# esi-neuroscience/syncopy

Measured on AMD Instinct MI355X. Metric: trials/sec for mtmfft+coherence (256 ch x 4096 samples, 7 DPSS tapers, full CSD), higher is better.
Workload: dtype f32 transforms; CSD operands fp16 hi+lo (22-bit), f32 accumulate; 1 GPU; BASELINE configs[2]: connectivityanalysis method='coh', AR(2) AnalogData, 256 ch x 4096 samp x 1000 trials per GPU, tapsmofrq=1 Hz (7 DPSS tapers), polyremoval=0, output='abs', inputs resident in HBM; trials_per_gpu=1000, channels=256, samples=4096, tapers=7, freqs=2049, batch=1000, fft_kernel=mtmfft_quad_kernel<12, 2, 2, false> + seq_mean_kernel

## Files before the change

include/spyhip.h:

```cpp
#ifndef SPYHIP_H
#define SPYHIP_H

#include <stddef.h>
#include <stdint.h>

#ifdef __cplusplus
extern "C" {
#endif

typedef struct spyhip_ctx spyhip_ctx;
typedef struct spyhip_fft_plan spyhip_fft_plan;
typedef struct spyhip_cwt_plan spyhip_cwt_plan;
typedef struct spyhip_queue spyhip_queue;

enum spyhip_output {
    SPYHIP_OUT_POW = 0,
    SPYHIP_OUT_ABS = 1,
    SPYHIP_OUT_FOURIER = 2,
    SPYHIP_OUT_REAL = 3,
    SPYHIP_OUT_IMAG = 4,
    SPYHIP_OUT_ANGLE = 5,
    SPYHIP_OUT_ABSREAL = 6,
    SPYHIP_OUT_ABSIMAG = 7
};

enum spyhip_detrend { SPYHIP_DETREND_NONE = -1, SPYHIP_DETREND_CONSTANT = 0, SPYHIP_DETREND_LINEAR = 1 };

int spyhip_version(void);
const char* spyhip_last_error(void);
int spyhip_ctx_create(int device, spyhip_ctx** ctx);
int spyhip_ctx_destroy(spyhip_ctx* ctx);
int spyhip_ctx_trim(spyhip_ctx* ctx);
int spyhip_ctx_set_stream(spyhip_ctx* ctx, void* stream);
int spyhip_ctx_synchronize(spyhip_ctx* ctx);

int spyhip_alloc(spyhip_ctx* ctx, size_t bytes, void** ptr_d);
int spyhip_free(spyhip_ctx* ctx, void* ptr_d);
int spyhip_memset(spyhip_ctx* ctx, void* ptr_d, int value, size_t bytes);
int spyhip_upload(spyhip_ctx* ctx, void* dst_d, const void* src, size_t bytes);
int spyhip_download(spyhip_ctx* ctx, void* dst, const void* src_d, size_t bytes);

int spyhip_queue_upload(spyhip_ctx* ctx, const float* data, int64_t nrows, int nchan, const int64_t* sampleinfo,
                        int ntrials, spyhip_queue** queue);
int spyhip_queue_destroy(spyhip_queue* queue);
const float* spyhip_queue_data(const spyhip_queue* queue);
int spyhip_queue_segments(const spyhip_queue* queue, const int64_t** start_d, const int64_t** stop_d, int* ntrials);

#define SPYHIP_UNIQUE_ID_BYTES 128
int spyhip_comm_unique_id(void* id_out);
int spyhip_comm_init(spyhip_ctx* ctx, const void* id, int rank, int nranks);
int spyhip_comm_destroy(spyhip_ctx* ctx);
int spyhip_comm_info(const spyhip_ctx* ctx, int* rank, int* nranks);
int spyhip_allreduce_csd(spyhip_ctx* ctx, void* acc_d, int nfreq, int nchan);
int spyhip_allreduce(spyhip_ctx* ctx, void* buf_d, int64_t n, int dtype);

int spyhip_fft_plan_create(spyhip_ctx* ctx, int nsig, int nfft, int nchan, int ntaper,
                           const double* tapers, double scale, int detrend, int demean_taper,
                           const int32_t* freq_idx, int nfsel, int output, int keeptapers,
                           spyhip_fft_plan** plan);
int spyhip_fft_plan_destroy(spyhip_fft_plan* plan);
int spyhip_fft_exec(spyhip_fft_plan* plan, const float* data_d, int64_t ld,
                    const int32_t* chan_idx_d, const int64_t* seg_start_d, const int64_t* seg_lo_d,
                    const int64_t* seg_hi_d, int nseg, void* out_d);
int spyhip_fft_plan_set_blocked(spyhip_fft_plan* plan, int on);
int spyhip_fft_plan_set_precision(spyhip_fft_plan* plan, int reference);
int spyhip_fft_plan_set_reference_mean(spyhip_fft_plan* plan, int on);
int spyhip_fft_plan_set_absmax(spyhip_fft_plan* plan, float* absmax_d);
const char* spyhip_fft_plan_kernel_name(const spyhip_fft_plan* plan);

int spyhip_csd_accumulate(spyhip_ctx* ctx, const void* spec_d, int64_t nrows, int nfreq, int nchan,
                          void* acc_d);
int spyhip_csd_set_phase_exact(spyhip_ctx* ctx, int on);
int spyhip_csd_accumulate_split(spyhip_ctx* ctx, const void* spec_d, int64_t nrows, int nfreq, int nchan,
                                void* acc_d, const float* absmax_d);
int spyhip_csd_accumulate_split_range(spyhip_ctx* ctx, const void* spec_d, int64_t nrows, int nfreq, int nchan,
                                      void* acc_d, const float* absmax_d, int f0, int nf);
int spyhip_csd_split_fallbacks(spyhip_ctx* ctx, int* count);
int spyhip_csd_accumulate_blocked(spyhip_ctx* ctx, const void* spec_d, int64_t nrows, int nfreq, int nchan,
                                  void* acc_d);
int spyhip_csd_tril_pack(spyhip_ctx* ctx, const void* acc_d, int nfreq, int nchan, void* packed_d);
int spyhip_csd_tril_unpack(spyhip_ctx* ctx, const void* packed_d, int nfreq, int nchan, void* acc_d);
int spyhip_csd_finalize(spyhip_ctx* ctx, void* acc_d, int nfreq, int nchan, double scale);

int spyhip_coh_normalize(spyhip_ctx* ctx, const void* csd_d, int nfreq, int nchan, int output,
                         void* out_d);

int spyhip_coh_from_accumulator(spyhip_ctx* ctx, const void* acc_d, int nfreq, int nchan, double scale, int output,
                                void* out_d);

int spyhip_cwt_plan_create_sl(spyhip_ctx* ctx, int nsig, int nchan, int nscales, const double* scales, double dt,
                              double cycles, double k_sd, int detrend, int output, const int32_t* tpos, int ntime_out,
                              spyhip_cwt_plan** out);
int spyhip_slt_combine(spyhip_ctx* ctx, void* acc_d, const void* spec_d, int64_t nrows, int nscales, int nsub, int s0,
                       int nchan, const double* expo, int init, int modulus_only);
int spyhip_spec_convert(spyhip_ctx* ctx, const void* in_d, int64_t n, int output, void* out_d);

int spyhip_ppc_accumulate(spyhip_ctx* ctx, const void* spec_d, int ntrials, int ntaper, int nfreq, int nchan,
                          void* acc_d);
int spyhip_ppc_accumulate_csd(spyhip_ctx* ctx, const void* csd_d, int ntrials, int64_t nelem, void* acc_d);
int spyhip_ppc_finalize(spyhip_ctx* ctx, const void* acc_d, int nfreq, int ni, int nj, int lower_only,
                        int64_t ntrials, void* out_d);

int spyhip_jack_coh_accumulate(spyhip_ctx* ctx, const void* spec_d, int ntrials, int ntaper, int nfreq, int nchan,
                               const void* csd_d, const void* direct_d, int output, int64_t ntrials_total,
                               void* sum_d, void* sum_d2);

int spyhip_ccov_nfft(int nsamples);
int spyhip_ccov_from_accumulator(spyhip_ctx* ctx, const void* acc_d, int nfft, int nchan, int nsamples, double scale,
                                 int norm, void* out_d);
int spyhip_ccov_normalize(spyhip_ctx* ctx, void* cc_d, int nlag, int nchan);

int spyhip_cwt_plan_create(spyhip_ctx* ctx, int nsig, int nchan, int nscales, const double* scales,
                           double dt, double w0, int detrend, int output, const int32_t* tpos,
                           int ntime_out, spyhip_cwt_plan** plan);
int spyhip_cwt_plan_create_family(spyhip_ctx* ctx, int nsig, int nchan, int nscales, const double* scales,
                                  double dt, int family, double p0, double p1, int detrend, int output,
                                  const int32_t* tpos, int ntime_out, spyhip_cwt_plan** plan);
int spyhip_cwt_plan_destroy(spyhip_cwt_plan* plan);
int spyhip_cwt_plan_set_precision(spyhip_cwt_plan* plan, int reference);
// ... 65 lines not shown
```

syncopy_amd/_lib.py:

```python
import ctypes as C
import os

HERE = os.path.dirname(os.path.abspath(__file__))
LIB_PATH = os.path.join(HERE, "libspyhip.so")

_lib = None

c_i32p = C.POINTER(C.c_int32)
c_i64p = C.POINTER(C.c_int64)
c_f32p = C.POINTER(C.c_float)
c_f64p = C.POINTER(C.c_double)
vp = C.c_void_p

SIGNATURES = {
    "spyhip_version": (C.c_int, []),
    "spyhip_last_error": (C.c_char_p, []),
    "spyhip_ctx_create": (C.c_int, [C.c_int, C.POINTER(vp)]),
    "spyhip_ctx_destroy": (C.c_int, [vp]),
    "spyhip_ctx_set_stream": (C.c_int, [vp, vp]),
    "spyhip_ctx_trim": (C.c_int, [vp]),
    "spyhip_ctx_synchronize": (C.c_int, [vp]),
    "spyhip_alloc": (C.c_int, [vp, C.c_size_t, C.POINTER(vp)]),
    "spyhip_free": (C.c_int, [vp, vp]),
    "spyhip_memset": (C.c_int, [vp, vp, C.c_int, C.c_size_t]),
    "spyhip_upload": (C.c_int, [vp, vp, vp, C.c_size_t]),
    "spyhip_download": (C.c_int, [vp, vp, vp, C.c_size_t]),
    "spyhip_queue_upload": (C.c_int, [vp, vp, C.c_int64, C.c_int, c_i64p, C.c_int, C.POINTER(vp)]),
    "spyhip_queue_destroy": (C.c_int, [vp]),
    "spyhip_queue_data": (vp, [vp]),
    "spyhip_queue_segments": (C.c_int, [vp, C.POINTER(vp), C.POINTER(vp), C.POINTER(C.c_int)]),
    "spyhip_comm_unique_id": (C.c_int, [vp]),
    "spyhip_comm_init": (C.c_int, [vp, vp, C.c_int, C.c_int]),
    "spyhip_comm_destroy": (C.c_int, [vp]),
    "spyhip_comm_info": (C.c_int, [vp, C.POINTER(C.c_int), C.POINTER(C.c_int)]),
    "spyhip_allreduce_csd": (C.c_int, [vp, vp, C.c_int, C.c_int]),
    "spyhip_allreduce": (C.c_int, [vp, vp, C.c_int64, C.c_int]),
    "spyhip_fft_plan_set_precision": (C.c_int, [vp, C.c_int]),
    "spyhip_cwt_plan_set_precision": (C.c_int, [vp, C.c_int]),
    "spyhip_cwt_plan_set_direct": (C.c_int, [vp, C.c_int]),
    "spyhip_fft_plan_set_reference_mean": (C.c_int, [vp, C.c_int]),
    "spyhip_fft_plan_create": (C.c_int, [vp, C.c_int, C.c_int, C.c_int, C.c_int, c_f64p, C.c_double, C.c_int,
                                         C.c_int, c_i32p, C.c_int, C.c_int, C.c_int, C.POINTER(vp)]),
    "spyhip_fft_plan_destroy": (C.c_int, [vp]),
    "spyhip_fft_exec": (C.c_int, [vp, vp, C.c_int64, vp, vp, vp, vp, C.c_int, vp]),
    "spyhip_fft_plan_kernel_name": (C.c_char_p, [vp]),
    "spyhip_fft_plan_set_blocked": (C.c_int, [vp, C.c_int]),
    "spyhip_csd_accumulate": (C.c_int, [vp, vp, C.c_int64, C.c_int, C.c_int, vp]),
    "spyhip_csd_set_phase_exact": (C.c_int, [vp, C.c_int]),
    "spyhip_csd_accumulate_split": (C.c_int, [vp, vp, C.c_int64, C.c_int, C.c_int, vp, vp]),
    "spyhip_csd_accumulate_split_range": (C.c_int, [vp, vp, C.c_int64, C.c_int, C.c_int, vp, vp, C.c_int, C.c_int]),
    "spyhip_csd_split_fallbacks": (C.c_int, [vp, C.POINTER(C.c_int)]),
    "spyhip_fft_plan_set_absmax": (C.c_int, [vp, vp]),
    "spyhip_csd_accumulate_blocked": (C.c_int, [vp, vp, C.c_int64, C.c_int, C.c_int, vp]),
    "spyhip_coh_from_accumulator": (C.c_int, [vp, vp, C.c_int, C.c_int, C.c_double, C.c_int, vp]),
    "spyhip_ppc_accumulate": (C.c_int, [vp, vp, C.c_int, C.c_int, C.c_int, C.c_int, vp]),
    "spyhip_ppc_accumulate_csd": (C.c_int, [vp, vp, C.c_int, C.c_int64, vp]),
    "spyhip_ppc_finalize": (C.c_int, [vp, vp, C.c_int, C.c_int, C.c_int, C.c_int, C.c_int64, vp]),
    "spyhip_jack_coh_accumulate": (C.c_int, [vp, vp, C.c_int, C.c_int, C.c_int, C.c_int, vp, vp, C.c_int, C.c_int64,
                                             vp, vp]),
    "spyhip_ccov_nfft": (C.c_int, [C.c_int]),
    "spyhip_ccov_normalize": (C.c_int, [vp, vp, C.c_int, C.c_int]),
    "spyhip_ccov_from_accumulator": (C.c_int, [vp, vp, C.c_int, C.c_int, C.c_int, C.c_double, C.c_int, vp]),
    "spyhip_csd_tril_pack": (C.c_int, [vp, vp, C.c_int, C.c_int, vp]),
    "spyhip_csd_tril_unpack": (C.c_int, [vp, vp, C.c_int, C.c_int, vp]),
    "spyhip_csd_finalize": (C.c_int, [vp, vp, C.c_int, C.c_int, C.c_double]),
    "spyhip_coh_normalize": (C.c_int, [vp, vp, C.c_int, C.c_int, C.c_int, vp]),
    "spyhip_cwt_plan_create": (C.c_int, [vp, C.c_int, C.c_int, C.c_int, c_f64p, C.c_double, C.c_double, C.c_int,
                                         C.c_int, c_i32p, C.c_int, C.POINTER(vp)]),
    "spyhip_cwt_plan_create_sl": (C.c_int, [vp, C.c_int, C.c_int, C.c_int, c_f64p, C.c_double, C.c_double,
                                            C.c_double, C.c_int, C.c_int, c_i32p, C.c_int, C.POINTER(vp)]),
    "spyhip_cwt_plan_create_family": (C.c_int, [vp, C.c_int, C.c_int, C.c_int, c_f64p, C.c_double, C.c_int, C.c_double,
                                                C.c_double, C.c_int, C.c_int, c_i32p, C.c_int, C.POINTER(vp)]),
    "spyhip_slt_combine": (C.c_int, [vp, vp, vp, C.c_int64, C.c_int, C.c_int, C.c_int, C.c_int, c_f64p, C.c_int,
                                     C.c_int]),
    "spyhip_spec_convert": (C.c_int, [vp, vp, C.c_int64, C.c_int, vp]),
    "spyhip_cwt_plan_destroy": (C.c_int, [vp]),
    "spyhip_cwt_exec": (C.c_int, [vp, vp, C.c_int64, vp, vp, vp, vp, C.c_int, vp, C.c_int]),
    "spyhip_granger": (C.c_int, [vp, vp, C.c_int, C.c_int, C.c_double, C.c_int, C.c_double, C.c_double, vp, vp, vp,
                                 c_f64p]),
    "spyhip_granger_last_iterations": (C.c_int, [vp]),
    "spyhip_wilson_cond": (C.c_int, [vp, vp, C.c_int, C.c_int, C.c_double, vp, vp, c_f64p]),
    "spyhip_wilson_init": (C.c_int, [vp, vp, C.c_int, C.c_int, C.c_int, C.c_int, vp, vp]),
    "spyhip_wilson_psi0": (C.c_int, [vp, vp, C.c_int, C.c_int, vp, vp]),
    "spyhip_wilson_g": (C.c_int, [vp, vp, vp, C.c_int, C.c_int, C.c_int, vp, vp]),
    "spyhip_wilson_plus": (C.c_int, [vp, vp, C.c_int, C.c_int64, vp, vp]),
    "spyhip_wilson_update": (C.c_int, [vp, vp, vp, vp, vp, vp, C.c_int, C.c_int, vp, c_f64p]),
    "spyhip_wilson_finish": (C.c_int, [vp, vp, vp, vp, C.c_int, C.c_int, vp, vp, vp, vp]),
    "spyhip_trial_mean_f32": (C.c_int, [vp, vp, vp, C.c_int64, C.c_int64]),
    "spyhip_trial_mean_c64": (C.c_int, [vp, vp, vp, C.c_int64, C.c_int64]),
    "spyhip_axis_nanmean": (C.c_int, [vp, vp, C.c_int64, C.c_int64, C.c_int64, C.c_int, vp]),
    "spyhip_trial_sum": (C.c_int, [vp, vp, vp, C.c_int64, C.c_int64]),
    "spyhip_trial_sum_finalize": (C.c_int, [vp, vp, vp, C.c_int64, C.c_int64, C.c_int]),
    "spyhip_trial_sqdev": (C.c_int, [vp, vp, vp, vp, C.c_int64, C.c_int64, C.c_int]),
# ... 50 lines not shown
```

syncopy_amd/backend.py:

```python
import ctypes as C
import os

import numpy as np
import torch

from . import _lib
from ._lib import SpyHipError, check

OUTPUT_KIND = {"pow": 0, "abs": 1, "fourier": 2, "complex": 2, "real": 3, "imag": 4, "angle": 5,
               "absreal": 6, "absimag": 7}
DETREND = {None: -1, False: -1, 0: 0, 1: 1}

_contexts = {}
_NP_DTYPE = {torch.float32: np.float32, torch.float64: np.float64, torch.complex64: np.complex64,
             torch.complex128: np.complex128, torch.int32: np.int32, torch.int64: np.int64, torch.uint8: np.uint8}


def require_gpu():
    if not torch.cuda.is_available():
        raise SpyHipError("no HIP device visible: syncopy_amd has no CPU fallback (torch.cuda.is_available() is False)")


class Context:

# ... 299 lines not shown
    for ctx in _contexts.values():
        ctx.lib.spyhip_ctx_trim(ctx.handle)
    if torch.cuda.is_available():
        torch.cuda.empty_cache()


def handover_buffer(shape, device, dtype=torch.complex64):
    key = (tuple(shape), str(device), dtype)
    buf = _handover.get(key)
    if buf is None:
        _handover.clear()
        buf = torch.empty(shape, dtype=dtype, device=device)
        _handover[key] = buf
    return buf


USE_BLOCKED_HANDOVER = False


class FFTPlan:

    def __init__(self, nsig, nfft, nchan, tapers, scale, detrend=None, demean_taper=False, freq_idx=None,
                 output="pow", keeptapers=True, device=None, reference_mean=False):
        self.ctx = context(device)
        tapers = np.ascontiguousarray(np.atleast_2d(tapers), dtype=np.float64)
        assert tapers.shape[1] == nsig, (tapers.shape, nsig)
        self.nsig, self.nfft, self.nchan, self.ntaper = int(nsig), int(nfft), int(nchan), tapers.shape[0]
        self.output = output
        self.kind = OUTPUT_KIND[output]
        self.keeptapers = bool(keeptapers)
        nf = self.nfft // 2 + 1
        if freq_idx is None:
            fi_p, self.nfsel = None, nf
        else:
            fi = np.ascontiguousarray(freq_idx, dtype=np.int32)
            fi_p, self.nfsel = fi.ctypes.data_as(_lib.c_i32p), int(fi.size)
        h = C.c_void_p()
        self.ctx.bind_stream()
        check(self.ctx.lib.spyhip_fft_plan_create(
            self.ctx.handle, self.nsig, self.nfft, self.nchan, self.ntaper,
            tapers.ctypes.data_as(_lib.c_f64p), float(scale), DETREND[detrend], int(bool(demean_taper)),
            fi_p, self.nfsel, self.kind, int(self.keeptapers), C.byref(h)), "spyhip_fft_plan_create")
        self.handle = h
        self.kout = self.ntaper if self.keeptapers else 1
        self.out_dtype = torch.complex64 if self.kind == 2 else torch.float32
        self.blocked = False
        self.reference_mean = int(reference_mean)
        if self.reference_mean:
            check(self.ctx.lib.spyhip_fft_plan_set_reference_mean(self.handle, self.reference_mean),
                  "spyhip_fft_plan_set_reference_mean")

    def set_precision(self, reference=True):
        return self.ctx.lib.spyhip_fft_plan_set_precision(self.handle, int(bool(reference))) == 0

    def set_blocked(self, on=True):
        rc = self.ctx.lib.spyhip_fft_plan_set_blocked(self.handle, int(bool(on)))
        if rc == 0:
            self.blocked = bool(on)
        return rc == 0

    @property
    def kernel_name(self):
        return self.ctx.lib.spyhip_fft_plan_kernel_name(self.handle).decode()

    def out_shape(self, nseg):
        if self.blocked:
            return (nseg * self.kout, (self.nchan + 3) // 4, self.nfsel, 4)
        return (nseg, self.kout, self.nfsel, self.nchan)

    def execute(self, data, seg_start, seg_lo=None, seg_hi=None, chan_idx=None, out=None, absmax=None):
        assert data.is_cuda and data.dtype == torch.float32 and data.dim() == 2 and data.is_contiguous()
        dev = data.device
        nseg = int(seg_start.numel())
        if seg_lo is None:
            seg_lo = seg_start
        if seg_hi is None:
            seg_hi = seg_start + self.nsig
        for t in (seg_start, seg_lo, seg_hi):
            assert t.is_cuda and t.dtype == torch.int64 and t.is_contiguous() and t.numel() == nseg
        if chan_idx is not None:
            assert chan_idx.is_cuda and chan_idx.dtype == torch.int32 and chan_idx.numel() == self.nchan
        else:
            assert data.shape[1] >= self.nchan
        if out is None:
            out = torch.empty(self.out_shape(nseg), dtype=self.out_dtype, device=dev)
        else:
            assert out.is_cuda and out.is_contiguous() and out.dtype == self.out_dtype
            assert tuple(out.shape) == self.out_shape(nseg), (tuple(out.shape), self.out_shape(nseg))
        self.ctx.bind_stream()
        tracked = False
        if absmax is not None:
            assert absmax.is_cuda and absmax.dtype == torch.float32 and absmax.numel() == self.nchan and absmax.is_contiguous()
            tracked = self.ctx.lib.spyhip_fft_plan_set_absmax(self.handle, _ptr(absmax)) == 0
        self.tracked_absmax = tracked
        try:
            check(self.ctx.lib.spyhip_fft_exec(self.handle, _ptr(data), int(data.shape[1]), _ptr(chan_idx),
                                               _ptr(seg_start), _ptr(seg_lo), _ptr(seg_hi), nseg, _ptr(out)),
                  "spyhip_fft_exec")
        finally:
            if self.tracked_absmax:
                self.ctx.lib.spyhip_fft_plan_set_absmax(self.handle, None)
        out.spyhip_absmax_tracked = self.tracked_absmax
        return out

    def __del__(self):
        try:
# ... 716 lines not shown
```

syncopy_amd/csrc/mtmfft.hip:

```cpp
#include <algorithm>
#include <cmath>
#include <cstdlib>
#include <string>

#include "spy_common.h"
#include "host_fft.h"
#include "mtmfft_kernel.h"
#include "mtmfft2_kernel.h"
#include "mtmfft_blue_kernel.h"
#include "mtmfft_long.h"
#include "mtmfft_generic.h"
#include "mtmfft_mixed_plan.h"

namespace spyfft {
}
#include "f64_stockham.h"
#include "mtmfft_f64_args.h"
namespace spyfft {
int dec64_launch_a(hipStream_t stream, const F64Args& a, int nfft, int npairs, int outk, bool mean);
int dec64_launch_b(hipStream_t stream, const F64Args& a, int nfft, int npairs, int outk, bool mean);
int dec64_launch_c(hipStream_t stream, const F64Args& a, int nfft, int npairs, int outk, bool mean);
int dec64_launch_d(hipStream_t stream, const F64Args& a, int nfft, int npairs, int outk, bool mean);
int dec64_launch_e(hipStream_t stream, const F64Args& a, int nfft, int npairs, int outk, bool mean);
int dec64_launch_f(hipStream_t stream, const F64Args& a, int nfft, int npairs, int outk, bool mean);
// ... 3 lines not shown
int dec64_launch_j(hipStream_t stream, const F64Args& a, int nfft, int npairs, int outk, bool mean);
int dec64_launch_k(hipStream_t stream, const F64Args& a, int nfft, int npairs, int outk, bool mean);
int dec64_launch_l(hipStream_t stream, const F64Args& a, int nfft, int npairs, int outk, bool mean);
int dec64_launch_m(hipStream_t stream, const F64Args& a, int nfft, int npairs, int outk, bool mean);
int dec64_launch_n(hipStream_t stream, const F64Args& a, int nfft, int npairs, int outk, bool mean);
int dec64_launch_half_a(hipStream_t stream, const F64Args& a, int nfft, int nchan, int outk, bool mean);
int dec64_launch_half_b(hipStream_t stream, const F64Args& a, int nfft, int nchan, int outk, bool mean);
struct Long64Args {
    MtmArgs m;
    const double* tapers64;
    const double2* twM;
    const double2* twN;
    const double2* twP;
    double2* scratch;
    const double* stats;
    const double* wsum;
    int seg0, nsegc;
    int npair;
};
int declong64_group(int M);
int declong64_launch_sub_a(hipStream_t stream, const Long64Args& a, int M, int P, long long nblocks);
int declong64_launch_sub_b(hipStream_t stream, const Long64Args& a, int M, int P, long long nblocks);
int declong64_launch_post(hipStream_t stream, const Long64Args& a, int P, int M, int outk, bool mean);
int f64_any_launch(hipStream_t stream, F64Args a, long long grid, long long chunk, int outk, bool mean);
int dec_launch_a(hipStream_t stream, const MtmArgs& a, int nfft, int nquads, int outk, bool mean);
int dec_launch_b(hipStream_t stream, const MtmArgs& a, int nfft, int nquads, int outk, bool mean);
int dec_launch_c(hipStream_t stream, const MtmArgs& a, int nfft, int nquads, int outk, bool mean);
int dec_launch_d(hipStream_t stream, const MtmArgs& a, int nfft, int nquads, int outk, bool mean);
int dec_launch_e(hipStream_t stream, const MtmArgs& a, int nfft, int nquads, int outk, bool mean);
int dec_launch_f(hipStream_t stream, const MtmArgs& a, int nfft, int nquads, int outk, bool mean);
int dec_launch_g(hipStream_t stream, const MtmArgs& a, int nfft, int nquads, int outk, bool mean);
int dec_launch_h(hipStream_t stream, const MtmArgs& a, int nfft, int nquads, int outk, bool mean);
int dec_launch_i(hipStream_t stream, const MtmArgs& a, int nfft, int nquads, int outk, bool mean);
int dec_launch_j(hipStream_t stream, const MtmArgs& a, int nfft, int nquads, int outk, bool mean);
int dec_launch_k(hipStream_t stream, const MtmArgs& a, int nfft, int nquads, int outk, bool mean);
int dec_launch_l(hipStream_t stream, const MtmArgs& a, int nfft, int nquads, int outk, bool mean);
int dec_launch_c2(hipStream_t stream, const MtmArgs& a, int nquads);
int dec_launch_half_a(hipStream_t stream, const MtmArgs& a, int nfft, int npairs, int outk, bool mean);
int dec_launch_half_b(hipStream_t stream, const MtmArgs& a, int nfft, int npairs, int outk, bool mean);
int dec_launch_half_c(hipStream_t stream, const MtmArgs& a, int nfft, int npairs, int outk, bool mean);
int quad_half_launch(hipStream_t stream, const MtmArgs& a, int npairs, int outk, bool mean);
int declong_group(int M);
int declong_launch_sub_a(hipStream_t stream, const LongArgs& a, int M, int P, long long nblocks);
int declong_launch_sub_b(hipStream_t stream, const LongArgs& a, int M, int P, long long nblocks);
int declong_launch_post(hipStream_t stream, const LongArgs& a, int P, int M, int outk, bool mean);
int mixed_launch(hipStream_t stream, const MtmArgs& a, const MixPlan& g, int threads, size_t lds, unsigned grid, int outk,
                 bool mean);
}

using spyfft::GenPlan;
using spyfft::MtmArgs;

struct spyhip_fft_plan {
    spyhip_ctx* ctx = nullptr;
    int nsig = 0, nfft = 0, nchan = 0, ntaper = 0, nfsel = 0, output = 0, keeptapers = 1;
    int detrend = -1, demean_taper = 0;
    float scale = 1.f;
    bool pow2 = false;
    bool dec = false;
    bool half = false;
    spy::DevBuf<float2> twh;
    bool mixed = false;
    spyfft::MixPlan mix{};
    int mix_threads = 0;
    bool blue = false;
    bool longp = false;
    bool long_direct = false;
    int dl_P = 0, dl_M = 0;
    int l1 = 0, l2 = 0;
    spy::DevBuf<float2> tw1, tw2, twM;
    spy::DevBuf<double> wsum, stats, stats_part;
    spy::DevBuf<float4> scratch;
    size_t stats_cap = 0, scratch_cap = 0;
    int log2n = 0, G = 1;
    GenPlan gen{};
    size_t lds_bytes = 0;
    spy::DevBuf<float> tapers;
    spy::DevBuf<float> tapers_half;
    spy::DevBuf<float2> tw, chirp, bhat;
    spy::DevBuf<int> fpos;
    bool identity_freq = true;
    bool blocked = false;
    unsigned* absmax = nullptr;
    float wnorm = 0.f;
    bool precision64 = false;
    bool f64_any = false;
    bool f64_dec = false;
    int f64_blue = 0;
    bool f64_dl = false;
    bool f64_half = false;
    spy::DevBuf<double2> tw64h;
    spy::DevBuf<double2> tw64_sub, tw64_P, scratch64;
    size_t scratch64_cap = 0;
    spy::DevBuf<double2> chirp64, bhat64;
    spywil::PlusPlan f64_plan{};
    spy::DevBuf<double2> f64_work;
    long long f64_chunk = 0;
    spy::DevBuf<double> tapers64;
    spy::DevBuf<double2> tw64;
    std::string fp32_kernel_name;
    bool ref_mean = false;
    bool seg_f64 = false;
    spy::DevBuf<float> means;
    size_t means_cap = 0;
    spy::DevBuf<float2> xpair;
    size_t xpair_cap = 0;
    std::string kernel_name;
};

namespace {

const double PI = 3.14159265358979323846264338327950288;

std::vector<float2> twiddle_table(int n) {
    std::vector<float2> t(n);
    for (int m = 0; m < n; ++m) {
        const double ang = -2.0 * PI * (double)m / (double)n;
        t[m] = make_float2((float)std::cos(ang), (float)std::sin(ang));
    }
    return t;
}

bool factorize(int n, int* radix, int* nfac) {
    static const int cand[] = {16, 8, 4, 2, 3, 5, 7, 11, 13};
    int k = 0;
    for (int c : cand) {
        while (n % c == 0 && n > 1) {
            if (k >= spyfft::GEN_MAXFAC) return false;
            radix[k++] = c;
            n /= c;
        }
    }
    *nfac = k;
    return n == 1;
}

template <int LOG2N, int G, int OUTK, bool MEAN>
int launch_quad(const spyhip_fft_plan* p, const MtmArgs& a, unsigned grid) {
    using C = spyfft::Cfg2<LOG2N, G>;
    auto kern = spyfft::mtmfft_quad_kernel<LOG2N, G, OUTK, MEAN>;
    SPY_HIP_CHECK(hipFuncSetAttribute(reinterpret_cast<const void*>(kern),
                                      hipFuncAttributeMaxDynamicSharedMemorySize, (int)C::LDS_BYTES));
    MtmArgs b = a;
    b.tapers = p->tapers_half.p;
    if (!b.tapers) { spy::set_error("fft_exec: plan without the pre-scaled taper table"); return -1; }
    hipLaunchKernelGGL(kern, dim3(grid), dim3(C::NTHREADS), C::LDS_BYTES, p->ctx->stream, b);
    SPY_HIP_CHECK(hipGetLastError());
    return 0;
}

template <int LOG2N, int G>
int launch_quad_mode(const spyhip_fft_plan* p, const MtmArgs& a, unsigned grid) {
    const bool mean = !p->keeptapers;
    const int outk = p->output == SPYHIP_OUT_FOURIER ? 2 : (p->output == SPYHIP_OUT_POW ? 0 : 1);
    switch (outk * 2 + (mean ? 1 : 0)) {
        case 0: return launch_quad<LOG2N, G, 0, false>(p, a, grid);
        case 1: return launch_quad<LOG2N, G, 0, true>(p, a, grid);
// ... 441 lines not shown
                    const long long q = (n * n) % (2LL * nfft);
                    const double ang = PI * (double)q / (double)nfft;
                    chirp[n] = make_double2(std::cos(ang), -std::sin(ang));
                    br[n] = std::cos(ang);
                    bi[n] = std::sin(ang);
                    if (n > 0) { br[M - n] = br[n]; bi[M - n] = bi[n]; }
                }
                spy::fft_host(br, bi);
                std::vector<double2> bhat(M);
                for (int i = 0; i < M; ++i) bhat[i] = make_double2(br[i] / M, bi[i] / M);
                if (p->chirp64.upload(chirp, p->ctx->stream) || p->bhat64.upload(bhat, p->ctx->stream)) return -2;
            }
        }
    }
    if (!p->tw64.p) {
        std::vector<double2> t(twlen);
        for (int m = 0; m < twlen; ++m) {
            const double ang = -2.0 * PI * (double)m / (double)twlen;
            t[m] = make_double2(std::cos(ang), std::sin(ang));
        }
        if (p->tw64.upload(t, p->ctx->stream)) return -2;
    }
    if (!p->precision64) p->fp32_kernel_name = p->kernel_name;
    p->precision64 = true;
    char buf[128];
    if (p->f64_half)
        std::snprintf(buf, sizeof buf, "mtmfft_dec64_kernel<HALF of N = %d, %d, %s>", p->nfft,
                      p->output == SPYHIP_OUT_FOURIER ? 2 : (p->output == SPYHIP_OUT_POW ? 0 : 1), p->keeptapers ? "false" : "true");
    else if (p->f64_dl)
        std::snprintf(buf, sizeof buf, "declong64_kernel<%d x %d, %d, %s>", p->dl_P, p->dl_M,
                      p->output == SPYHIP_OUT_FOURIER ? 2 : (p->output == SPYHIP_OUT_POW ? 0 : 1), p->keeptapers ? "false" : "true");
    else if (p->f64_dec)
        std::snprintf(buf, sizeof buf, "mtmfft_dec64_kernel<N = %d, %d, %s>", p->nfft,
                      p->output == SPYHIP_OUT_FOURIER ? 2 : (p->output == SPYHIP_OUT_POW ? 0 : 1), p->keeptapers ? "false" : "true");
    else if (p->f64_blue)
        std::snprintf(buf, sizeof buf, "mtmfft_f64_any_kernel<%d, %s> N=%d (Bluestein, M = %d)",
                      p->output == SPYHIP_OUT_FOURIER ? 2 : (p->output == SPYHIP_OUT_POW ? 0 : 1), p->keeptapers ? "false" : "true",
                      p->nfft, p->f64_blue);
    else
        std::snprintf(buf, sizeof buf, "mtmfft_f64_any_kernel<%d, %s> N=%d",
                      p->output == SPYHIP_OUT_FOURIER ? 2 : (p->output == SPYHIP_OUT_POW ? 0 : 1), p->keeptapers ? "false" : "true",
                      p->nfft);
    p->kernel_name = buf;
    return 0;
}

extern "C" int spyhip_fft_plan_set_reference_mean(spyhip_fft_plan* p, int on) {
    if (!p) { spy::set_error("fft_plan_set_reference_mean: null plan"); return -1; }
    p->ref_mean = on == 1;
    p->seg_f64 = on == 2;
    return 0;
}

extern "C" const char* spyhip_fft_plan_kernel_name(const spyhip_fft_plan* p) {
    return p ? p->kernel_name.c_str() : "";
}

extern "C" int spyhip_fft_exec(spyhip_fft_plan* p, const float* data_d, int64_t ld, const int32_t* chan_idx_d,
                               const int64_t* seg_start_d, const int64_t* seg_lo_d, const int64_t* seg_hi_d,
                               int nseg, void* out_d) {
    if (!p || !data_d || !seg_start_d || !seg_lo_d || !seg_hi_d || !out_d) { spy::set_error("fft_exec: null argument"); return -1; }
    if (nseg <= 0) return 0;
    SPY_HIP_CHECK(hipSetDevice(p->ctx->device));
    MtmArgs a{};
    a.data = data_d; a.ld = ld; a.chan_idx = chan_idx_d;
    a.seg_start = reinterpret_cast<const long long*>(seg_start_d);
    a.seg_lo = reinterpret_cast<const long long*>(seg_lo_d);
    a.seg_hi = reinterpret_cast<const long long*>(seg_hi_d);
    a.nseg = nseg; a.nsig = p->nsig; a.nchan = p->nchan; a.ntaper = p->ntaper;
    a.tapers = p->tapers.p; a.tw = p->tw.p; a.scale = p->scale;
    a.detrend = p->detrend; a.demean_taper = p->demean_taper;
    a.fpos = p->identity_freq ? nullptr : p->fpos.p;
    a.nfsel = p->nfsel; a.out_kind = p->output; a.out = out_d;
    a.blocked = p->blocked ? 1 : 0;
    a.means = nullptr;
    a.seg_f64 = p->seg_f64 ? 1 : 0;
    a.absmax = (p->absmax && !p->blocked) ? p->absmax : nullptr;
    a.wnorm = p->wnorm;
    if (a.absmax && !(p->pow2 && p->log2n <= 13 && !p->precision64)) {
        const int bt = std::min(256, ((p->nchan + 63) / 64) * 64);
        const int ncb = (p->nchan + bt - 1) / bt;
        for (int s0 = 0; s0 < nseg; s0 += 65535) {
            MtmArgs m = a;
            m.seg_start += s0; m.seg_lo += s0; m.seg_hi += s0;
            hipLaunchKernelGGL(spyfft::seg_range_kernel, dim3(ncb, std::min(65535, nseg - s0)), dim3(bt), 0, p->ctx->stream, m);
        }
        SPY_HIP_CHECK(hipGetLastError());
        a.absmax = nullptr;
    }
    if (p->ref_mean && p->detrend == 0) {
        const size_t need = (size_t)nseg * p->nchan;
        if (need > p->means_cap) {
            if (p->means.p) { SPY_HIP_CHECK(hipStreamSynchronize(p->ctx->stream)); (void)hipFree(p->means.p); p->means.p = nullptr; }
            if (p->means.alloc(need)) return -2;
            p->means_cap = need;
        }
        const int bt = std::min(256, ((p->nchan + 63) / 64) * 64);
        const int ncb = (p->nchan + bt - 1) / bt;
        for (int s0 = 0; s0 < nseg; s0 += 65535) {
            MtmArgs m = a;
            m.seg_start += s0; m.seg_lo += s0; m.seg_hi += s0;
            const int ns = std::min(65535, nseg - s0);
            hipLaunchKernelGGL(spyfft::seq_mean_kernel, dim3(ncb, ns), dim3(bt), 0, p->ctx->stream, m,
                               p->means.p + (size_t)s0 * p->nchan);
        }
        SPY_HIP_CHECK(hipGetLastError());
        a.means = p->means.p;
    }
    const int npairs = (p->nchan + 1) / 2;
    if (p->precision64) {
        spyfft::F64Args fa{};
        fa.m = a;
        fa.tapers64 = p->tapers64.p;
        fa.tw64 = p->tw64.p;
        fa.scale64 = (double)p->scale;
        const long long grid = (long long)nseg * npairs;
        const int outk64 = p->output == SPYHIP_OUT_FOURIER ? 2 : (p->output == SPYHIP_OUT_POW ? 0 : 1);
        if (p->f64_half) {
            fa.tw64 = p->tw64h.p;
            fa.tw64_full = p->tw64.p;
            int rc;
            if ((rc = spyfft::dec64_launch_half_a(p->ctx->stream, fa, p->nfft, p->nchan, outk64, !p->keeptapers)) != -100) return rc;
            if ((rc = spyfft::dec64_launch_half_b(p->ctx->stream, fa, p->nfft, p->nchan, outk64, !p->keeptapers)) != -100) return rc;
            spy::set_error("fft_exec: no half-length reference-precision schedule for nfft = %d", p->nfft);
            return -1;
        }
        if (p->f64_dl) {
            spyfft::Long64Args L{};
            a.nfft = p->nfft;
            L.m = a;
            L.tapers64 = p->tapers64.p;
            L.twM = p->tw64_sub.p; L.twN = p->tw64.p; L.twP = p->tw64_P.p;
            L.wsum = p->wsum.p;
            L.npair = npairs;
            const size_t N = (size_t)p->nfft;
            const size_t nstat = (size_t)nseg * p->nchan * (2 + p->ntaper);
            const int nz = p->demean_taper ? p->ntaper + 1 : 1;
            if (nstat > p->stats_cap) {
                if (p->stats.p) { (void)hipFree(p->stats.p); p->stats.p = nullptr; }
                if (p->stats_part.p) { (void)hipFree(p->stats_part.p); p->stats_part.p = nullptr; }
                if (p->stats.alloc(nstat) ||
                    p->stats_part.alloc((size_t)nseg * (p->ntaper + 1) * spyfft::LONG_SPLITS * p->nchan * 2)) return -2;
                p->stats_cap = nstat;
            }
            L.stats = p->stats.p;
            if ((p->detrend >= 0 && !(p->detrend == 0 && a.means)) || p->demean_taper) {
                if (nseg > 65535 || nz * spyfft::LONG_SPLITS > 65535) { spy::set_error("fft_exec: too many segments / tapers per call"); return -1; }
                hipLaunchKernelGGL(spyfft::long_stats_kernel, dim3((p->nchan + 63) / 64, nseg, nz * spyfft::LONG_SPLITS),
                                   dim3(256), 0, p->ctx->stream, a, p->stats_part.p, nz);
                hipLaunchKernelGGL(spyfft::long_stats_final_kernel, dim3((unsigned)(((size_t)nseg * p->nchan + 255) / 256)), dim3(256),
                                   0, p->ctx->stream, a, p->stats_part.p, nz, p->stats.p);
                SPY_HIP_CHECK(hipGetLastError());
            }
            const size_t per_seg = (size_t)npairs * p->ntaper * N;
            size_t chunk = std::max<size_t>(1, std::min<size_t>((size_t)nseg, (((size_t)2 << 30) / sizeof(double2)) / std::max<size_t>(per_seg, 1)));
            if (chunk * per_seg > p->scratch64_cap) {
                if (p->scratch64.p) { (void)hipFree(p->scratch64.p); p->scratch64.p = nullptr; }
                if (p->scratch64.alloc(chunk * per_seg)) return -2;
                p->scratch64_cap = chunk * per_seg;
            }
// ... 257 lines not shown
            L.nsegc = std::min<int>((int)chunk, nseg - s0);
            const long long items = (long long)L.nsegc * L.nquad * p->ntaper;
            int rc = launch_long(p->ctx, L, p->l1, 0, items);
            if (!rc) rc = launch_long(p->ctx, L, p->l2, 1, items);
            if (!rc && !L.direct) rc = launch_long(p->ctx, L, p->l1, 2, items);
            if (rc) return rc;
            switch (outk * 2 + (mean ? 1 : 0)) {
                case 0: rc = launch_long_post<0, false>(p->ctx, L); break;
                case 1: rc = launch_long_post<0, true>(p->ctx, L); break;
                case 2: rc = launch_long_post<1, false>(p->ctx, L); break;
                case 3: rc = launch_long_post<1, true>(p->ctx, L); break;
                case 4: rc = launch_long_post<2, false>(p->ctx, L); break;
                default: rc = launch_long_post<2, true>(p->ctx, L); break;
            }
            if (rc) return rc;
        }
        return 0;
    }
    if (p->blue) {
        a.nfft = p->nfft; a.chirp = p->chirp.p; a.bhat = p->bhat.p;
        const int G = p->G;
        const int nitem = (p->nchan + 3) / 4;
        a.npg = (nitem + G - 1) / G;
        int S = 8 / G; if (S < 1) S = 1; if (S > a.npg) S = a.npg;
        a.S = S;
        a.ncl = (a.npg + S - 1) / S;
        const long long nclusters = (long long)nseg * a.ncl;
        const long long grid = ((nclusters + 7) / 8) * S * 8;
        if (grid > 0x7fffffffLL) { spy::set_error("fft_exec: grid too large (%lld blocks)", grid); return -1; }
        const unsigned g = (unsigned)grid;
        switch (p->log2n) {
            case 8: return launch_blue_mode<8, 16>(p, a, g);
            case 9: return launch_blue_mode<9, 8>(p, a, g);
            case 10: return launch_blue_mode<10, 4>(p, a, g);
            case 11: return launch_blue_mode<11, 2>(p, a, g);
            case 12: return launch_blue_mode<12, 1>(p, a, g);
            case 13: return launch_blue_mode<13, 1>(p, a, g);
            default: spy::set_error("no Bluestein kernel for M=2^%d", p->log2n); return -1;
        }
    }
    const long long grid = (long long)nseg * npairs;
    if (grid > 0x7fffffffLL) { spy::set_error("fft_exec: grid too large (%lld blocks)", grid); return -1; }
    const bool mean = !p->keeptapers;
    const int outk = p->output == SPYHIP_OUT_FOURIER ? 2 : (p->output == SPYHIP_OUT_POW ? 0 : 1);
    switch (outk * 2 + (mean ? 1 : 0)) {
        case 0: return launch_generic<0, false>(p, a, (unsigned)grid);
        case 1: return launch_generic<0, true>(p, a, (unsigned)grid);
        case 2: return launch_generic<1, false>(p, a, (unsigned)grid);
        case 3: return launch_generic<1, true>(p, a, (unsigned)grid);
        case 4: return launch_generic<2, false>(p, a, (unsigned)grid);
        default: return launch_generic<2, true>(p, a, (unsigned)grid);
    }
}
```

Baseline: 49130 trials/s.

## Overlap per-segment mean pass with FFT via chunked side stream

Splits the segment batch into chunks and runs the reference-mean kernel for each chunk on a dedicated non-blocking side stream. Each chunk's transform waits on an event, so the mean pass for later chunks can overlap the FFT of earlier ones instead of running serially in front of the whole batch. The chunk size is derived from CU count and wave geometry, and the path is skipped under graph capture. It adds extra launches and event synchronisation per chunk and shortens each FFT grid, which may hurt occupancy.

```diff
diff --git a/include/spyhip.h b/include/spyhip.h
--- a/include/spyhip.h
+++ b/include/spyhip.h
@@ -65,6 +65,7 @@
 int spyhip_fft_plan_set_blocked(spyhip_fft_plan* plan, int on);
 int spyhip_fft_plan_set_precision(spyhip_fft_plan* plan, int reference);
 int spyhip_fft_plan_set_reference_mean(spyhip_fft_plan* plan, int on);
+int spyhip_fft_plan_set_mean_chunk(spyhip_fft_plan* plan, int nseg);
 int spyhip_fft_plan_set_absmax(spyhip_fft_plan* plan, float* absmax_d);
 const char* spyhip_fft_plan_kernel_name(const spyhip_fft_plan* plan);
 
diff --git a/syncopy_amd/_lib.py b/syncopy_amd/_lib.py
--- a/syncopy_amd/_lib.py
+++ b/syncopy_amd/_lib.py
@@ -39,6 +39,7 @@
     "spyhip_cwt_plan_set_precision": (C.c_int, [vp, C.c_int]),
     "spyhip_cwt_plan_set_direct": (C.c_int, [vp, C.c_int]),
     "spyhip_fft_plan_set_reference_mean": (C.c_int, [vp, C.c_int]),
+    "spyhip_fft_plan_set_mean_chunk": (C.c_int, [vp, C.c_int]),
     "spyhip_fft_plan_create": (C.c_int, [vp, C.c_int, C.c_int, C.c_int, C.c_int, c_f64p, C.c_double, C.c_int,
                                          C.c_int, c_i32p, C.c_int, C.c_int, C.c_int, C.POINTER(vp)]),
     "spyhip_fft_plan_destroy": (C.c_int, [vp]),
diff --git a/syncopy_amd/backend.py b/syncopy_amd/backend.py
--- a/syncopy_amd/backend.py
+++ b/syncopy_amd/backend.py
@@ -375,6 +375,10 @@
 
     def set_precision(self, reference=True):
         return self.ctx.lib.spyhip_fft_plan_set_precision(self.handle, int(bool(reference))) == 0
+
+    def set_mean_chunk(self, nseg):
+        check(self.ctx.lib.spyhip_fft_plan_set_mean_chunk(self.handle, -1 if nseg is None else int(nseg)),
+              "spyhip_fft_plan_set_mean_chunk")
 
     def set_blocked(self, on=True):
         rc = self.ctx.lib.spyhip_fft_plan_set_blocked(self.handle, int(bool(on)))
diff --git a/syncopy_amd/csrc/mtmfft.hip b/syncopy_amd/csrc/mtmfft.hip
--- a/syncopy_amd/csrc/mtmfft.hip
+++ b/syncopy_amd/csrc/mtmfft.hip
@@ -79,6 +79,7 @@
 using spyfft::MtmArgs;
 
 struct spyhip_fft_plan {
+    static constexpr int MEAN_EVENTS = 16;
     spyhip_ctx* ctx = nullptr;
     int nsig = 0, nfft = 0, nchan = 0, ntaper = 0, nfsel = 0, output = 0, keeptapers = 1;
     int detrend = -1, demean_taper = 0;
@@ -130,6 +131,17 @@
     bool seg_f64 = false;
     spy::DevBuf<float> means;
     size_t means_cap = 0;
+    int mean_chunk = 0;
+    hipStream_t side = nullptr;
+    hipEvent_t ev_entry = nullptr, ev_chunk[MEAN_EVENTS] = {};
+    ~spyhip_fft_plan() {
+        if (side) {
+            (void)hipStreamSynchronize(side);
+            (void)hipStreamDestroy(side);
+            (void)hipEventDestroy(ev_entry);
+            for (hipEvent_t e : ev_chunk) (void)hipEventDestroy(e);
+        }
+    }
     spy::DevBuf<float2> xpair;
     size_t xpair_cap = 0;
     std::string kernel_name;
@@ -677,16 +689,45 @@
     return 0;
 }
 
+extern "C" int spyhip_fft_plan_set_mean_chunk(spyhip_fft_plan* p, int nseg) {
+    if (!p) { spy::set_error("fft_plan_set_mean_chunk: null plan"); return -1; }
+    p->mean_chunk = nseg < 0 ? -1 : nseg;
+    return 0;
+}
+
 extern "C" const char* spyhip_fft_plan_kernel_name(const spyhip_fft_plan* p) {
     return p ? p->kernel_name.c_str() : "";
 }
 
-extern "C" int spyhip_fft_exec(spyhip_fft_plan* p, const float* data_d, int64_t ld, const int32_t* chan_idx_d,
-                               const int64_t* seg_start_d, const int64_t* seg_lo_d, const int64_t* seg_hi_d,
-                               int nseg, void* out_d) {
-    if (!p || !data_d || !seg_start_d || !seg_lo_d || !seg_hi_d || !out_d) { spy::set_error("fft_exec: null argument"); return -1; }
-    if (nseg <= 0) return 0;
-    SPY_HIP_CHECK(hipSetDevice(p->ctx->device));
+namespace {
+
+int reserve_means(spyhip_fft_plan* p, int nseg) {
+    const size_t need = (size_t)nseg * p->nchan;
+    if (need > p->means_cap) {
+        if (p->means.p) { SPY_HIP_CHECK(hipStreamSynchronize(p->ctx->stream)); (void)hipFree(p->means.p); p->means.p = nullptr; }
+        p->means_cap = 0;
+        if (p->means.alloc(need)) return -2;
+        p->means_cap = need;
+    }
+    return 0;
+}
+
+int launch_seq_mean(const spyhip_fft_plan* p, const MtmArgs& a, float* means, hipStream_t stream) {
+    const int bt = std::min(256, ((p->nchan + 63) / 64) * 64);
+    const int ncb = (p->nchan + bt - 1) / bt;
+    for (int s0 = 0; s0 < a.nseg; s0 += 65535) {
+        MtmArgs m = a;
+        m.seg_start += s0; m.seg_lo += s0; m.seg_hi += s0;
+        const int ns = std::min(65535, a.nseg - s0);
+        hipLaunchKernelGGL(spyfft::seq_mean_kernel, dim3(ncb, ns), dim3(bt), 0, stream, m, means + (size_t)s0 * p->nchan);
+    }
+    SPY_HIP_CHECK(hipGetLastError());
+    return 0;
+}
+
+int exec_range(spyhip_fft_plan* p, const float* data_d, int64_t ld, const int32_t* chan_idx_d,
+               const int64_t* seg_start_d, const int64_t* seg_lo_d, const int64_t* seg_hi_d,
+               int nseg, void* out_d, const float* means_ready) {
     MtmArgs a{};
     a.data = data_d; a.ld = ld; a.chan_idx = chan_idx_d;
     a.seg_start = reinterpret_cast<const long long*>(seg_start_d);
@@ -714,23 +755,13 @@
         a.absmax = nullptr;
     }
     if (p->ref_mean && p->detrend == 0) {
-        const size_t need = (size_t)nseg * p->nchan;
-        if (need > p->means_cap) {
-            if (p->means.p) { SPY_HIP_CHECK(hipStreamSynchronize(p->ctx->stream)); (void)hipFree(p->means.p); p->means.p = nullptr; }
-            if (p->means.alloc(need)) return -2;
-            p->means_cap = need;
-        }
-        const int bt = std::min(256, ((p->nchan + 63) / 64) * 64);
-        const int ncb = (p->nchan + bt - 1) / bt;
-        for (int s0 = 0; s0 < nseg; s0 += 65535) {
-            MtmArgs m = a;
-            m.seg_start += s0; m.seg_lo += s0; m.seg_hi += s0;
-            const int ns = std::min(65535, nseg - s0);
-            hipLaunchKernelGGL(spyfft::seq_mean_kernel, dim3(ncb, ns), dim3(bt), 0, p->ctx->stream, m,
-                               p->means.p + (size_t)s0 * p->nchan);
-        }
-        SPY_HIP_CHECK(hipGetLastError());
-        a.means = p->means.p;
+        if (means_ready) {
+            a.means = means_ready;
+        } else {
+            if (int rc = reserve_means(p, nseg)) return rc;
+            if (int rc = launch_seq_mean(p, a, p->means.p, p->ctx->stream)) return rc;
+            a.means = p->means.p;
+        }
     }
     const int npairs = (p->nchan + 1) / 2;
     if (p->precision64) {
@@ -1094,3 +1125,102 @@
         default: return launch_generic<2, true>(p, a, (unsigned)grid);
     }
 }
+
+constexpr int MEAN_SPLIT = 8, MEAN_MIN_ROUNDS = 4;
+
+int mean_chunk_of(const spyhip_fft_plan* p, int nseg) {
+    if (!(p->ref_mean && p->detrend == 0)) return 0;
+    int L = p->mean_chunk;
+    if (const char* e = std::getenv("SPYHIP_MEAN_CHUNK")) {
+        char* end = nullptr;
+        const long v = std::strtol(e, &end, 10);
+        if (end != e && v >= 0 && v <= 0x7fffffffL) L = (int)v;
+    }
+    if (L < 0) {
+        if (!(p->pow2 && p->log2n <= 13 && !p->precision64)) return 0;
+        const int npg = ((p->nchan + 3) / 4 + p->G - 1) / p->G;
+        const int S = std::max(1, std::min(8 / p->G, npg));
+        const long long wps = (long long)((npg + S - 1) / S) * S;
+        const long long cu = std::max(1, p->ctx->num_cu);
+        long long g = wps, r = cu;
+        while (r) { const long long t = g % r; g = r; r = t; }
+        const long long whole = cu / g;
+        const long long lmin = (MEAN_MIN_ROUNDS * cu + wps - 1) / wps;
+        long long l = std::max<long long>(lmin, (nseg + MEAN_SPLIT - 1) / MEAN_SPLIT);
+        l = (l + whole - 1) / whole * whole;
+        L = l > 0x7fffffffLL ? 0 : (int)l;
+    }
+    return (L <= 0 || L >= nseg) ? 0 : L;
+}
+
+int exec_forked(spyhip_fft_plan* p, const float* data_d, int64_t ld, const int32_t* chan_idx_d,
+                const int64_t* seg_start_d, const int64_t* seg_lo_d, const int64_t* seg_hi_d,
+                int nseg, void* out_d, int L) {
+    hipStream_t caller = p->ctx->stream;
+    if (!p->side) {
+        hipStream_t s = nullptr;
+        SPY_HIP_CHECK(hipStreamCreateWithFlags(&s, hipStreamNonBlocking));
+        hipEvent_t ev[spyhip_fft_plan::MEAN_EVENTS + 1] = {};
+        for (hipEvent_t& e : ev) {
+            if (hipEventCreateWithFlags(&e, hipEventDisableTiming) != hipSuccess) {
+                for (hipEvent_t d : ev) if (d) (void)hipEventDestroy(d);
+                (void)hipStreamDestroy(s);
+                spy::set_error("fft_exec: cannot create the events of the mean pass's stream");
+                return -2;
+            }
+        }
+        p->ev_entry = ev[0];
+        for (int i = 0; i < spyhip_fft_plan::MEAN_EVENTS; ++i) p->ev_chunk[i] = ev[i + 1];
+        p->side = s;
+    }
+    if (int rc = reserve_means(p, nseg)) return rc;
+    SPY_HIP_CHECK(hipEventRecord(p->ev_entry, caller));
+    SPY_HIP_CHECK(hipStreamWaitEvent(p->side, p->ev_entry, 0));
+    const size_t kout = p->keeptapers ? (size_t)p->ntaper : 1;
+    const size_t seg_bytes = p->blocked ? kout * (size_t)((p->nchan + 3) / 4) * p->nfsel * 32
+                                        : kout * (size_t)p->nfsel * p->nchan * (p->output == SPYHIP_OUT_FOURIER ? 8 : 4);
+    int rc = 0, c = 0;
+    hipEvent_t last = p->ev_entry;
+    for (int s0 = 0; s0 < nseg && !rc; s0 += L, ++c) {
+        const int ns = std::min(L, nseg - s0);
+        float* means = p->means.p + (size_t)s0 * p->nchan;
+        MtmArgs m{};
+        m.data = data_d; m.ld = ld; m.chan_idx = chan_idx_d;
+        m.seg_start = reinterpret_cast<const long long*>(seg_start_d) + s0;
+        m.seg_lo = reinterpret_cast<const long long*>(seg_lo_d) + s0;
+        m.seg_hi = reinterpret_cast<const long long*>(seg_hi_d) + s0;
+        m.nseg = ns; m.nsig = p->nsig; m.nchan = p->nchan;
+        rc = launch_seq_mean(p, m, means, p->side);
+        if (rc) break;
+        last = p->ev_chunk[c % spyhip_fft_plan::MEAN_EVENTS];
+        if (hipEventRecord(last, p->side) != hipSuccess || hipStreamWaitEvent(caller, last, 0) != hipSuccess) {
+            spy::set_error("fft_exec: cannot order the transform behind its mean pass");
+            rc = -1;
+            break;
+        }
+        rc = exec_range(p, data_d, ld, chan_idx_d, seg_start_d + s0, seg_lo_d + s0, seg_hi_d + s0, ns,
+                        reinterpret_cast<char*>(out_d) + (size_t)s0 * seg_bytes, means);
+    }
+    if (rc) {
+        if (hipEventRecord(last, p->side) == hipSuccess) (void)hipStreamWaitEvent(caller, last, 0);
+    }
+    return rc;
+}
+
+}
+
+extern "C" int spyhip_fft_exec(spyhip_fft_plan* p, const float* data_d, int64_t ld, const int32_t* chan_idx_d,
+                               const int64_t* seg_start_d, const int64_t* seg_lo_d, const int64_t* seg_hi_d,
+                               int nseg, void* out_d) {
+    if (!p || !data_d || !seg_start_d || !seg_lo_d || !seg_hi_d || !out_d) { spy::set_error("fft_exec: null argument"); return -1; }
+    if (nseg <= 0) return 0;
+    SPY_HIP_CHECK(hipSetDevice(p->ctx->device));
+    int L = mean_chunk_of(p, nseg);
+    if (L) {
+        hipStreamCaptureStatus st = hipStreamCaptureStatusNone;
+        if (hipStreamIsCapturing(p->ctx->stream, &st) != hipSuccess) { (void)hipGetLastError(); L = 0; }
+        else if (st != hipStreamCaptureStatusNone) L = 0;
+    }
+    if (L) return exec_forked(p, data_d, ld, chan_idx_d, seg_start_d, seg_lo_d, seg_hi_d, nseg, out_d, L);
+    return exec_range(p, data_d, ld, chan_idx_d, seg_start_d, seg_lo_d, seg_hi_d, nseg, out_d, nullptr);
+}
```

New measurement: 48600 trials/s. 1.1% lower.
